# RenYurui/Global-Flow-Local-Attention

Hardware: AMD Instinct MI355X
Metric: images/sec (fwd+bwd) PoseGenerator 256x176 attn_layer=2,3 -- feature-warping hot path (higher is better)
Workload: dtype f32 (FC products: 2-term f16 splits exact to 2^-24 on f16 MFMA, f32 accumulate)

## Files before the change

### global_flow_local_attention_amd/csrc/fc_block.hip

```cpp
#include "fc_gemm.h"

namespace gfla {

static int64_t align256(int64_t v) { return (v + 255) & ~(int64_t)255; }

enum { kAmaxSrc = 0, kAmaxTgt = 1, kAmaxW = 2, kAmaxZs = 3, kAmaxZt = 4, kAmaxSlots = 8 };

enum FcConv {
  kConvDirect,
  kConvDirect16,
  kConvWino32,
  kConvWino16,
};
enum FcWgrad {
  kWgradDirect32,
  kWgradDirect16,
  kWgradWino32,
  kWgradWino16,
};
static bool fc_wgrad_wino(FcWgrad w) { return w == kWgradWino32 || w == kWgradWino16; }

struct FcPlan {
  int split;
  bool scaled;
  FcConv fwd, dgrad;
  bool pack_wf, pack_wd;
  int pack_split;
  bool pack_uf, pack_ud;
  bool dgrads_together;
  FcWgrad wgrad;
  FcWgrad wgrad_both;
  bool wgrads_together;
  bool wgrad_x32;
  bool own_scatter;
};

static FcPlan fc_plan(int64_t B, int C, int H, int W, int k, int mode) {
  (void)C;
  FcPlan P;
  P.split = fc_base_mode(mode);
  P.scaled = P.split != 0 || mode == 5;
  P.fwd = mode == 4 ? kConvWino32 : mode == 5 ? (k == 5 ? kConvDirect16 : kConvWino16) : kConvDirect;
  P.dgrad = mode == 4 ? kConvWino32 : mode == 5 ? kConvDirect16 : kConvDirect;
  P.pack_wf = P.fwd == kConvDirect || P.fwd == kConvDirect16;
  P.pack_wd = P.dgrad == kConvDirect || P.dgrad == kConvDirect16;
  P.pack_split = P.dgrad == kConvDirect16 ? 2 : P.split;
  P.pack_uf = P.fwd == kConvWino32 || P.fwd == kConvWino16;
  P.pack_ud = P.dgrad == kConvWino32;
  P.dgrads_together = fc_is_wino(mode);
  P.wgrad_x32 = mode == 1 && k == 5;
  P.wgrad = fc_is_wino(mode) || P.wgrad_x32 ? (mode == 5 && k == 5 ? kWgradWino16 : kWgradWino32)
                                            : (P.split ? kWgradDirect16 : kWgradDirect32);
  P.wgrad_both = P.wgrad_x32 ? kWgradWino16 : P.wgrad;
  P.wgrads_together = tuning(GFLA_TUNE_WINO_LAUNCH) != 2;
  const FcHalf hs = fc_half(H, W, k, true);
  P.own_scatter = tuning(GFLA_TUNE_FC_SCATTER_ATOMICS) != 1 && fc_scatter_own_rows(B, hs.Ho, hs.Wo) >= 1;
  return P;
}

struct FcLayout {
  FcPlan plan;
  FcHalf hs, ht;
  int nch_c, cpad, nt_d, KK, dw1_tiles;
  int64_t amax, xs, xt, gs, hid, wd_t, wd_s, gt, wf_t, wf_s, wu_ft, wu_fs, wu_dt, wu_ds, fwd_total;
  int64_t dzs, dzt, dw_s, dw_t, zero_bytes, zs_pk, zt_pk, dxs, dxt, b0p, dw1p, red, red_tmp, dwp, dwp2, x32, x32b, bwd_total;
};

static FcLayout fc_layout(int64_t B, int C, int H, int W, int k, int mode) {
  const bool wino = fc_is_wino(mode);
  FcLayout L;
  L.plan = fc_plan(B, C, H, W, k, mode);
  const FcPlan &P = L.plan;
  L.hs = fc_half(H, W, k, true);
  L.ht = fc_half(H, W, k, false);
  L.nch_c = (int)ceil_div(C, kFcChunk);
  L.cpad = L.nch_c * kFcChunk;
  L.nt_d = (int)ceil_div(C, kFcTN);
  L.KK = k * k;
  const int nch_h = kFcHidden / kFcChunk;
  int64_t o = 0;
  auto take = [&](int64_t bytes) {
    const int64_t at = o;
    o += align256(bytes);
    return at;
  };
  L.amax = take(kAmaxSlots * 4);
  L.xs = take(fc_packed_bytes(B, L.nch_c, L.hs.Sx, P.split));
  L.xt = take(fc_packed_bytes(B, L.nch_c, L.ht.Sx, P.split));
  L.gs = take(B * L.hs.Mg * kFcHidden * 4);
  L.hid = take(B * (int64_t)H * W * kFcHidden * 4);
// ... 279 lines not shown
static int fc_fold_both(const FcLayout &L, const unsigned char *sc, float *g_source, float *g_target, int acc_s, int64_t B, int C,
                        int H, int W, hipStream_t stream) {
  return fc_fold2(reinterpret_cast<const float *>(sc + L.dxs), g_source, L.hs, L.hs.Mdg * (int64_t)C, acc_s,
                  reinterpret_cast<const float *>(sc + L.dxt), g_target, L.ht, L.ht.Mdg * (int64_t)C, 0, B, C, H, W, stream);
}

static int fc_unpack_wgrad_both(const FcLayout &L, const unsigned char *ws, unsigned char *sc, float *g_w0, int C, int k,
                                hipStream_t stream) {
  const uint32_t *a = reinterpret_cast<const uint32_t *>(ws + L.amax);
  return fc_unpack_wgrad(reinterpret_cast<float *>(sc + L.dw_t), reinterpret_cast<float *>(sc + L.dw_s), a + kAmaxTgt, a + kAmaxSrc,
                         a + kAmaxZt, a + kAmaxZs, g_w0, C, L.cpad, k, stream);
}

static int fc_backward(void *ws_, const float *flow, const float *w1, const float *g_logits, void *scratch_,
                       float *g_source, float *g_target, float *g_flow, float *g_w0, float *g_b0, float *g_w1,
                       float *g_b1, int64_t B, int C, int H, int W, int k, float slope, int mode_, int flags,
                       hipStream_t stream) {
  if (!ws_ || !flow || !w1 || !g_logits || !scratch_) return GFLA_ERR_NULL_POINTER;
  GFLA_TRY(fc_args_ok(B, C, H, W, k, mode_));
  if (B == 0) return GFLA_OK;
  note_path(mode_ == 5 ? GFLA_PATH_FC_BWD_MODE5 : GFLA_PATH_FC_BWD_MODE0 + mode_);
  const FcLayout L = fc_layout(B, C, H, W, k, mode_);
  const FcPlan &P = L.plan;
  unsigned char *ws = static_cast<unsigned char *>(ws_), *sc = static_cast<unsigned char *>(scratch_);
  uint32_t *amax = reinterpret_cast<uint32_t *>(ws + L.amax);
  const float *hid = reinterpret_cast<const float *>(ws + L.hid);
  float *red_tmp = reinterpret_cast<float *>(sc + L.red_tmp);
  const float *gs = reinterpret_cast<const float *>(ws + L.gs);
  const bool need_s = g_source || g_w0, need_t = g_target || g_w0;
  float *dzs = need_s ? reinterpret_cast<float *>(sc + L.dzs) : nullptr;
  float *dzt = need_t ? reinterpret_cast<float *>(sc + L.dzt) : nullptr;
  float *b0p = g_b0 ? reinterpret_cast<float *>(sc + L.b0p) : nullptr;
  const int64_t tiles = ceil_div((int64_t)H * W, 64);
  const bool own = need_s && need_t && P.own_scatter;
  if (hipMemsetAsync(sc + (own ? L.dzt : 0), 0, L.zero_bytes - (own ? L.dzt : 0), stream) != hipSuccess) return GFLA_ERR_LAUNCH;
  if ((P.scaled || own) && hipMemsetAsync(amax + kAmaxZs, 0, 8, stream) != hipSuccess) return GFLA_ERR_LAUNCH;
  GFLA_TRY(fc_sample_tail_bwd(gs, flow, hid, w1, g_logits, own ? nullptr : dzs, dzt, g_flow, b0p, B, H, W, k, L.hs.Mg * kFcHidden,
                              L.hs.Wo, L.hs.Wp, L.ht.Wp, L.hs.Sz * kFcHidden, L.ht.Sz * kFcHidden, L.hs.lead, L.ht.lead, slope,
                              flags & GFLA_FC_ACCUMULATE_FLOW, stream, own ? amax + kAmaxZt : nullptr));
  if (own)
    GFLA_TRY(fc_sample_scatter_own(flow, dzt, dzs, amax + kAmaxZt, amax + kAmaxZs, B, H, W, k, L.hs.Ho, L.hs.Wo, L.hs.Wp, L.ht.Wp,
                                   L.hs.Sz * kFcHidden, L.ht.Sz * kFcHidden, L.hs.lead, L.ht.lead, L.hs.Sz, stream));
  const float *dw1p = nullptr;
  if (g_w1 || g_b1) {
    float *part = reinterpret_cast<float *>(sc + L.dw1p);
    GFLA_TRY(fc_dw1(hid, g_logits, part, B, H * W, L.KK, L.dw1_tiles, slope, stream));
    dw1p = part;
  }
  GFLA_TRY(fc_reduce_bias_w1(b0p, B * tiles, g_b0, dw1p, B * L.dw1_tiles, g_w1, g_b1, L.KK, red_tmp, stream));
  const int acc_s = (flags & GFLA_FC_ACCUMULATE_SOURCE) ? 1 : 0;
  const bool both_x = g_source && g_target;
  const bool dgrads_done = P.dgrads_together && both_x;
  if (dgrads_done) {
    if (P.dgrad == kConvDirect16 && !own)
      GFLA_TRY(fc_maxabs_multi(dzs, B * L.hs.Sz * kFcHidden, amax + kAmaxZs, dzt, B * L.ht.Sz * kFcHidden, amax + kAmaxZt, nullptr,
                               0, nullptr, stream));
    GFLA_TRY(fc_dgrad_convs(L, ws, sc, true, true, B, C, k, stream));
    GFLA_TRY(fc_fold_both(L, sc, g_source, g_target, acc_s, B, C, H, W, stream));
  }
  const bool defer = g_w0 && P.wgrad != kWgradDirect16;
  const bool wgrads_done = defer && fc_wgrad_wino(P.wgrad) && both_x && P.wgrads_together;
  const bool z_both = P.split != 0 && need_s && need_t;
  if (z_both) {
    if (!own)
      GFLA_TRY(fc_maxabs_multi(dzs, B * L.hs.Sz * kFcHidden, amax + kAmaxZs, dzt, B * L.ht.Sz * kFcHidden, amax + kAmaxZt, nullptr,
                               0, nullptr, stream));
    GFLA_TRY(fc_pack_z2(dzs, amax + kAmaxZs, sc + L.zs_pk, L.hs.Sz, dzt, amax + kAmaxZt, sc + L.zt_pk, L.ht.Sz, B, kFcHidden,
                        P.split, stream));
// ... 154 lines not shown
```

### global_flow_local_attention_amd/csrc/fc_gemm.h

```cpp
#pragma once

#include "gfla_common.h"

namespace gfla {

typedef float f32x16 __attribute__((ext_vector_type(16)));
typedef _Float16 f16x8 __attribute__((ext_vector_type(8)));
typedef short s16x4 __attribute__((ext_vector_type(4)));
typedef short s16x8 __attribute__((ext_vector_type(8)));

constexpr int kFcChunk = 16;
constexpr int kFcTN = 128;
constexpr int kFcHidden = 128;

template <int MODE>
struct Fc;
template <>
struct Fc<0> {
  static constexpr int NS = 1, ESZ = 4, REC = 64, PIECES = 4, PITCH = 80, KB = 2;
};
template <>
struct Fc<1> {
  static constexpr int NS = 1, ESZ = 2, REC = 32, PIECES = 2, PITCH = 48, KB = 1;
};
template <>
struct Fc<2> {
  static constexpr int NS = 2, ESZ = 2, REC = 32, PIECES = 2, PITCH = 48, KB = 1;
};
template <>
struct Fc<3> {
  static constexpr int NS = 3, ESZ = 2, REC = 32, PIECES = 2, PITCH = 48, KB = 1;
};

inline bool fc_is_wino(int mode) { return mode == 4 || mode == 5; }
inline int fc_base_mode(int mode) { return fc_is_wino(mode) ? 0 : mode; }
inline int fc_nsplit(int mode) { return mode == 0 ? 1 : mode; }
inline int fc_esz(int mode) { return mode == 0 ? 4 : 2; }
inline bool fc_mode_ok(int mode) { return mode >= 0 && mode <= 5; }

struct PackedDesc {
  const unsigned char *base;
  int64_t split_stride;
  int64_t batch_stride;
  int64_t chunk_stride;
  int pix_stride;
};
// ... 172 lines not shown
```

### global_flow_local_attention_amd/csrc/fc_sample.hip

```cpp
#include "fc_gemm.h"
#include "lds_plane.h"

namespace gfla {

constexpr int kSmpPix = 64;
constexpr int kSmpPitch = kFcHidden + 1;

struct Corner {
  int i00, i01, i10, i11;
  int z00, z01, z10, z11;
  float xl, xr, yt, yb;
};

template <int KS>
__device__ __forceinline__ Corner corners(float fx, float fy, int x, int y, int H, int W, int wps, int wpz = 0) {
  constexpr int LO = KS / 2, HI = KS - 1 - LO;
  const float dx = fx + (float)x, dy = fy + (float)y;
  const float fdx = floorf(dx), fdy = floorf(dy);
  Corner c;
  c.xr = dx - fdx;
  c.xl = 1.f - c.xr;
  c.yb = dy - fdy;
  c.yt = 1.f - c.yb;
  const float cx = fminf(fmaxf(fdx, -(float)(HI + 1)), (float)(W + LO));
  const float cy = fminf(fmaxf(fdy, -(float)(HI + 1)), (float)(H + LO));
  const int qx = (int)cx, qy = (int)cy;
  const int gx0 = clampi(qx, -HI, W - 1 + LO) + HI, gx1 = clampi(qx + 1, -HI, W - 1 + LO) + HI;
  const int gy0 = clampi(qy, -HI, H - 1 + LO) + HI, gy1 = clampi(qy + 1, -HI, H - 1 + LO) + HI;
  c.i00 = gy0 * wps + gx0;
  c.i01 = gy0 * wps + gx1;
  c.i10 = gy1 * wps + gx0;
  c.i11 = gy1 * wps + gx1;
  c.z00 = gy0 * wpz + gx0;
  c.z01 = gy0 * wpz + gx1;
  c.z10 = gy1 * wpz + gx0;
  c.z11 = gy1 * wpz + gx1;
  return c;
}
// ... 166 lines not shown
    tp[0] = in ? hq[j].x : 0.f, tp[1] = in ? hq[j].y : 0.f, tp[2] = in ? hq[j].z : 0.f, tp[3] = in ? hq[j].w : 0.f;
  }
#pragma unroll
  for (int j = 0; j < NW; ++j) {
    const int i = t + 256 * j;
    if (i < kFcHidden * KK) w_s[i] = wq[j];
  }
  __syncthreads();
  {
    const int p = p0 + lane;
    const bool live = p < HW;
#pragma unroll
    for (int q = 0; q < KK; ++q) gl[q] = live ? gl[q] : 0.f;
    uint32_t mx = 0;
#pragma unroll 4
    for (int o = wave; o < kFcHidden; o += 4) {
      const float pre = tile[lane * kSmpPitch + o];
      const float *w = w_s + o * KK;
      float ga = 0.f;
#pragma unroll
      for (int q = 0; q < KK; ++q) ga = fmaf(w[q], gl[q], ga);
      const float gp = pre > 0.f ? ga : ga * slope;
      tile[lane * kSmpPitch + o] = gp;
      mx = max(mx, __float_as_uint(gp) & 0x7fffffffu);
    }
    if (amax_d) {
#pragma unroll
      for (int m = 32; m >= 1; m >>= 1) mx = max(mx, (uint32_t)__shfl_xor((int)mx, m));
      if (lane == 0 && mx > __hip_atomic_load(amax_d, __ATOMIC_RELAXED, __HIP_MEMORY_SCOPE_AGENT)) atomicMax(amax_d, mx);
    }
  }
  __syncthreads();
  const float *gsb = gs + b * gs_bs;
  float *zsb = dzs ? dzs + b * zs_bs : nullptr;
  float *ztb = dzt ? dzt + b * zt_bs : nullptr;
  float s0 = 0.f, s1 = 0.f;
  int pend_t = -1, pend_b = -1;
  float pt0 = 0.f, pt1 = 0.f, pb0 = 0.f, pb1 = 0.f;
  constexpr int kWalk = kSmpPix / 4;
  const int pw0 = p0 + wave * kWalk;
  const int nwalk = max(0, min(kWalk, HW - pw0));
  float fx_l = 0.f, fy_l = 0.f;
  if ((lane & (kWalk - 1)) < nwalk) {
    fx_l = flow[(b * 2 + 0) * HW + pw0 + (lane & (kWalk - 1))];
    fy_l = flow[(b * 2 + 1) * HW + pw0 + (lane & (kWalk - 1))];
  }
  if (amax_d && __any(!(fabsf(fx_l) < INFINITY) || !(fabsf(fy_l) < INFINITY))) {
    if (lane == 0) atomicMax(amax_d, 0x7fc00000u);
  }
  Corner cn;
  float gn[8];
  auto issue = [&](int it) {
    const int p = pw0 + it;
    const int y = p / W, x = p - y * W;
    const float fx = __int_as_float(__builtin_amdgcn_readlane(__float_as_int(fx_l), it));
    const float fy = __int_as_float(__builtin_amdgcn_readlane(__float_as_int(fy_l), it));
    cn = corners<KS>(fx, fy, x, y, H, W, wps, wpz);
    if (gflow) {
      const float *g00 = gsb + (int64_t)cn.i00 * kFcHidden + lane, *g01 = gsb + (int64_t)cn.i01 * kFcHidden + lane;
      const float *g10 = gsb + (int64_t)cn.i10 * kFcHidden + lane, *g11 = gsb + (int64_t)cn.i11 * kFcHidden + lane;
      gn[0] = g00[0], gn[1] = g01[0], gn[2] = g10[0], gn[3] = g11[0];
      gn[4] = g00[64], gn[5] = g01[64], gn[6] = g10[64], gn[7] = g11[64];
    }
  };
  if (!zsb) {
    float old_x = 0.f, old_y = 0.f, res_x = 0.f, res_y = 0.f;
    if (gflow && acc_flow && lane < nwalk) {
      old_x = gflow[(b * 2 + 0) * HW + pw0 + lane];
// ... 77 lines not shown
        atomic_add(zb, pb0); atomic_add(zb + 64, pb1);
      }
      float *z00 = zsb + (int64_t)(lead_s + c.z00) * kFcHidden + lane, *z10 = zsb + (int64_t)(lead_s + c.z10) * kFcHidden + lane;
      atomic_add(z00, lt0); atomic_add(z00 + 64, lt1);
      atomic_add(z10, lb0); atomic_add(z10 + 64, lb1);
      pend_t = c.z01, pend_b = c.z11;
      pt0 = wb * d0, pt1 = wb * d1, pb0 = wd * d0, pb1 = wd * d1;
    }
    if (gflow) {
      float gx = d0 * (c.yt * (g[1] - g[0]) + c.yb * (g[3] - g[2])) + d1 * (c.yt * (g[5] - g[4]) + c.yb * (g[7] - g[6]));
      float gy = d0 * (c.xl * (g[2] - g[0]) + c.xr * (g[3] - g[1])) + d1 * (c.xl * (g[6] - g[4]) + c.xr * (g[7] - g[5]));
      gx = wave_sum_lane63(gx);
      gy = wave_sum_lane63(gy);
      if (lane == 63) {
        float *fxp = gflow + (b * 2 + 0) * HW + p, *fyp = gflow + (b * 2 + 1) * HW + p;
        *fxp = acc_flow ? *fxp + gx : gx;
        *fyp = acc_flow ? *fyp + gy : gy;
      }
    }
  }
  if (zsb && pend_t >= 0) {
    float *zt = zsb + (int64_t)(lead_s + pend_t) * kFcHidden + lane, *zb = zsb + (int64_t)(lead_s + pend_b) * kFcHidden + lane;
    atomic_add(zt, pt0); atomic_add(zt + 64, pt1);
    atomic_add(zb, pb0); atomic_add(zb + 64, pb1);
  }
  if (b0_partials) {
    bsum[wave * kFcHidden + lane] = s0;
    bsum[wave * kFcHidden + lane + 64] = s1;
    __syncthreads();
    if (t < kFcHidden)
      b0_partials[(b * gridDim.x + blockIdx.x) * kFcHidden + t] =
          (bsum[t] + bsum[kFcHidden + t]) + (bsum[2 * kFcHidden + t] + bsum[3 * kFcHidden + t]);
  }
}

static int smp_check(int64_t B, int H, int W, int k) {
  if (B < 0 || H <= 0 || W <= 0) return GFLA_ERR_BAD_SHAPE;
  if (k != 3 && k != 5) return GFLA_ERR_UNSUPPORTED;
  if (B > 65535 || (int64_t)H * W > 0x3fffffffLL) return GFLA_ERR_UNSUPPORTED;
  return GFLA_OK;
}

int fc_sample_tail_fwd(const float *gs, const float *gt, const float *flow, const float *b0, const float *w1,
                       const float *b1, float *hid, float *logits, int64_t B, int H, int W, int k, int64_t gs_bs,
                       int64_t gt_bs, int wps, int wpt, float slope, hipStream_t stream) {
  if (!gs || !gt || !flow || !w1 || !hid || !logits) return GFLA_ERR_NULL_POINTER;
  if (int rc = smp_check(B, H, W, k)) return rc;
  if (B == 0) return GFLA_OK;
  const dim3 grid((unsigned)ceil_div((int64_t)H * W, kSmpPix), (unsigned)B);
  const unsigned lds = (unsigned)((kSmpPix * kSmpPitch + kFcHidden * k * k) * sizeof(float));
  if (k == 3)
    fc_tail_fwd_kernel<3><<<grid, 256, lds, stream>>>(gs, gt, flow, b0, w1, b1, hid, logits, H, W, gs_bs, gt_bs, wps, wpt, slope);
  else
    fc_tail_fwd_kernel<5><<<grid, 256, lds, stream>>>(gs, gt, flow, b0, w1, b1, hid, logits, H, W, gs_bs, gt_bs, wps, wpt, slope);
  return launch_status();
}

int fc_sample_tail_bwd(const float *gs, const float *flow, const float *hid, const float *w1, const float *g_logits,
                       float *dzs, float *dzt, float *gflow, float *b0_partials, int64_t B, int H, int W, int k,
                       int64_t gs_bs, int wps, int wpz, int wpt, int64_t zs_bs, int64_t zt_bs, int lead_s, int lead_t,
                       float slope, int acc_flow, hipStream_t stream, uint32_t *amax_d) {
  if (!gs || !flow || !hid || !w1 || !g_logits) return GFLA_ERR_NULL_POINTER;
  if (int rc = smp_check(B, H, W, k)) return rc;
  if (B == 0) return GFLA_OK;
  const dim3 grid((unsigned)ceil_div((int64_t)H * W, kSmpPix), (unsigned)B);
  const unsigned lds = (unsigned)((kSmpPix * kSmpPitch + kFcHidden * k * k + 4 * kFcHidden) * sizeof(float));
// ... 626 lines not shown
```

### global_flow_local_attention_amd/csrc/gs_route.h

```cpp
#pragma once

#include <type_traits>

#include "agg_stream.h"
#include "be_bwd_lds.h"
#include "be_fwd_pix.h"
#include "be_fwd_wrow.h"
#include "be_tile.h"

namespace gfla {

template <int LO, int HI, typename F>
inline void k_dispatch(int k, F &&f) {
  if constexpr (LO >= HI) {
    f(std::integral_constant<int, HI>{});
  } else {
    if (k == LO) f(std::integral_constant<int, LO>{});
    else k_dispatch<LO + 1, HI>(k, f);
  }
}
#define GFLA_K_SWITCH(NAME, LO, HI, KV, ...) \
  ::gfla::k_dispatch<LO, HI>(KV, [&](auto gfla_k_) { constexpr int NAME = decltype(gfla_k_)::value; __VA_ARGS__; })
#define GFLA_WIN_SWITCH(MARGIN, ...)                                   \
  do {                                                                 \
// ... 274 lines not shown

enum class AggGaPath { kUnsupported, kStream, kLds };
struct AggGaRoute {
  AggGaPath path;
  AggStreamPlan plan;
  int G, nsuper, CS, ntiles;
  int64_t blocks, padded;
  unsigned lds_bytes;
};
inline AggGaRoute agg_ga_route(int acc_size, int64_t B, int64_t C, int64_t Hs, int64_t Ws, int64_t H, int64_t W, int k) {
  AggGaRoute r{};
  if (acc_size == 4 && agg_stream_wanted(k) && agg_stream_shape_ok(B, C, Hs, Ws, k, false) &&
      agg_stream_plan(B, C, Hs, Ws, H, W, k, r.plan))
    return r.path = AggGaPath::kStream, r;
  const int64_t ntiles = ceil_div(H * W, 512);
  int64_t G = lds_budget() / (Hs * Ws * (int64_t)acc_size);
  if (G < 1) return r;
  if (G > C) G = C;
  int64_t nsuper = 1;
  while (B * ntiles * nsuper < 4 * kNumCU && nsuper * 2 * G <= C) nsuper *= 2;
  const int64_t CS = ceil_div(C, nsuper);
  nsuper = ceil_div(C, CS);
  if (G > CS) G = CS;
  r.G = (int)G, r.nsuper = (int)nsuper, r.CS = (int)CS, r.ntiles = (int)ntiles;
  r.blocks = B * nsuper * ntiles;
  r.padded = ceil_div(r.blocks, kNumXCD) * kNumXCD;
  r.lds_bytes = (unsigned)(G * Hs * Ws * acc_size);
  if (grid_ok(r.blocks)) r.path = AggGaPath::kLds;
  return r;
}
enum class AggBwdPath { kUnsupported, kLds, kGlobal };
struct AggBwdRoute {
  AggBwdPath path;
  bool product, lds_fallback;
  PlaneGeo scatter, fallback;
  Geo global;
};
inline AggBwdRoute agg_bwd_route(int elem_size, int acc_size, bool need_src, bool need_flow, bool need_logits, bool workspace,
                                 int64_t B, int64_t C, int64_t Hs, int64_t Ws, int64_t H, int64_t W, int k) {
  AggBwdRoute r{};
  const bool half = elem_size == 2, fit = scatter_gather_planes_fit(Hs, Ws, acc_size);
  r.product = elem_size == 4 && need_src && workspace && tuning(GFLA_TUNE_AGG) != 1 &&
              (Hs * Ws * (int64_t)acc_size <= lds_budget() || (!need_flow && !need_logits));
  r.lds_fallback = r.product && fit;
  if (r.lds_fallback) r.fallback = whole_plane_bwd_route(kGoutAttn, elem_size, acc_size, true, false, B, C, Hs, Ws, H, W, k);
  if ((tuning(GFLA_TUNE_AGG) != 1 || half) && fit) {
    r.path = AggBwdPath::kLds;
    if (need_src || need_flow) {
      r.scatter = whole_plane_bwd_route(kGoutAttn, elem_size, acc_size, need_src, need_flow, B, C, Hs, Ws, H, W, k);
      if (r.scatter.G == 0) r.path = AggBwdPath::kUnsupported;
    }
  } else if (!half) {
    r.global = chunk_geometry(B, C, H * W, 32, kHalfFillWaves);
    if (grid_ok(r.global.blocks)) r.path = AggBwdPath::kGlobal;
  }
  return r;
}

}
```

### global_flow_local_attention_amd/csrc/local_attn_aggregate.hip

```cpp
#include <type_traits>

#include "gfla_common.h"
#include "gs_route.h"
#include "patch_mfma.h"
#include "rs_taps.h"

namespace gfla {

template <typename A>
__device__ __forceinline__ A exp_t(A v);
template <>
__device__ __forceinline__ float exp_t<float>(float v) { return expf(v); }
template <>
__device__ __forceinline__ double exp_t<double>(double v) { return exp(v); }

template <typename A, int K>
struct PatchTaps {
  int xL[K], xR[K], yT[K], yB[K];
  A ax[K], ay[K];
  int x0, y0;
  bool dense;

  __device__ __forceinline__ void init(A fx0, A fy0, int xf, int yf, int Hs, int Ws) {
    dense = true;
// ... 978 lines not shown
                                                   pg.lds, stream, src, flow, gout, (float *)glogits,
                                                   gflow ? attn : (const T *)nullptr, (float *)gflow, (int)C, (int)Hs, (int)Ws,
                                                   (int)H, (int)W, pg.CH, pg.CS, pg.nsuper, pg.tgroups, pg.pitch, (int)r.plan.total,
                                                   pg.tw_log2, pg.ntile)));
    }
  } else {
    GFLA_K_SWITCH(K, 1, 5, k, agg_ga_lds_kernel<T, K><<<dim3((unsigned)r.padded), dim3(512), r.lds_bytes, stream>>>(
                                  src, flow, gout, glogits, gflow ? attn : nullptr, gflow, (int)C, (int)Hs, (int)Ws, (int)H, (int)W,
                                  r.G, r.nsuper, r.CS, r.ntiles, (int)r.blocks));
  }
  int st = launch_status();
  if (st == GFLA_OK && sm && glogits) {
    const int64_t n = B * H * W;
    GFLA_K_SWITCH(K, 1, 5, k, agg_softmax_bwd_kernel<T, K><<<dim3((unsigned)ceil_div(n, kBlock)), dim3(kBlock), 0, stream>>>(
                                  attn, glogits, n, (int)(H * W)));
    st = launch_status();
  }
  return st;
}

template <typename T>
static int launch_agg_scatter(const PlaneGeo &g, const T *src, const T *flow, const T *attn, const T *gout, T *gsrc,
                              typename Num<T>::acc *gflow, int64_t B, int64_t C, int64_t Hs, int64_t Ws, int64_t H, int64_t W, int k,
                              hipStream_t stream, const unsigned *skip_stat = nullptr, unsigned skip_limit = 0) {
  int st = GFLA_OK;
  GFLA_K_SWITCH(K, 1, 5, k, st = launch_be_bwd_lds<T, K>(kGoutAttn, g, src, flow, gout, attn, gsrc, gflow, B, C, Hs, Ws, H, W, stream,
                                                         0, 0, (const T *)nullptr, skip_stat, skip_limit));
  return st;
}

template <typename T>
static int aggregate_bwd(const T *src, const T *flow, const T *attn, const T *gout, T *gsrc,
                         typename Num<T>::acc *gflow, typename Num<T>::acc *glogits, int64_t B, int64_t C, int64_t Hs, int64_t Ws, int64_t H, int64_t W,
                         int k, int sm, gfla_stream_t stream_, void *workspace = nullptr) {
  if (!src || !flow || !attn || !gout) return GFLA_ERR_NULL_POINTER;
  int st = agg_check(B, C, Hs, Ws, H, W, k);
  if (st != GFLA_OK) return st;
  if (!gsrc && !gflow && !glogits) return GFLA_OK;
  hipStream_t stream = static_cast<hipStream_t>(stream_);
  using A = typename Num<T>::acc;
  const AggBwdRoute r = agg_bwd_route((int)sizeof(T), (int)sizeof(A), gsrc != nullptr, gflow != nullptr, glogits != nullptr,
                                      workspace != nullptr, B, C, Hs, Ws, H, W, k);
  if constexpr (std::is_same<T, float>::value) {
    if (r.product) {
      if (r.lds_fallback && r.fallback.G == 0) return GFLA_ERR_UNSUPPORTED;
      const unsigned *skip_stat = nullptr;
      unsigned skip_limit = 0;
      st = agg_source_bwd_mfma(flow, attn, gout, gsrc, workspace, B, C, Hs, Ws, H, W, k, 1, r.lds_fallback ? 1 : 0, &skip_stat,
                               &skip_limit, stream);
      if (st == GFLA_OK) {
        if (r.lds_fallback && skip_limit != 0xffffffffu) {
          st = launch_agg_scatter<T>(r.fallback, src, flow, attn, gout, gsrc, (A *)nullptr, B, C, Hs, Ws, H, W, k, stream, skip_stat,
                                     skip_limit);
          if (st != GFLA_OK) return st;
        }
        if (gflow || glogits) st = launch_agg_ga<T>(src, flow, attn, gout, glogits, gflow, B, C, Hs, Ws, H, W, k, sm, stream);
        return st;
      }
      if (st != GFLA_ERR_UNSUPPORTED) return st;
    }
  }
  switch (r.path) {
    case AggBwdPath::kUnsupported: return GFLA_ERR_UNSUPPORTED;
    case AggBwdPath::kLds:
      st = GFLA_OK;
      if (gsrc || gflow) st = launch_agg_scatter<T>(r.scatter, src, flow, attn, gout, gsrc, gflow, B, C, Hs, Ws, H, W, k, stream);
      if (st == GFLA_OK && glogits)
        st = launch_agg_ga<T>(src, flow, attn, gout, glogits, (A *)nullptr, B, C, Hs, Ws, H, W, k, sm, stream);
      return st;
    case AggBwdPath::kGlobal:
      if constexpr (sizeof(T) != 2) {
        const Geo &g = r.global;
        GFLA_K_SWITCH(K, 1, 5, k, agg_bwd_kernel<T, K><<<dim3((unsigned)g.blocks), dim3(kBlock), 0, stream>>>(
                                      src, flow, attn, gout, gsrc, gflow, glogits, (int)C, (int)Hs, (int)Ws, (int)H, (int)W, sm, g.cpt,
                                      g.ncg, g.sp_blocks));
      }
      return launch_status();
  }
  return st;
}

template <typename T>
static int local_attn_source_bwd(const T *src, const T *flow, const T *gunf, const T *attn, const T *gout,
                                 T *gsrc, typename Num<T>::acc *gflow, int64_t B, int64_t C, int64_t Hs, int64_t Ws, int64_t H,
                                 int64_t W, int k, int layout, gfla_stream_t stream_) {
  using A = typename Num<T>::acc;
  if (!src || !flow || (!gunf && !(attn && gout)) || ((attn == nullptr) != (gout == nullptr))) return GFLA_ERR_NULL_POINTER;
  int st = agg_check(B, C, Hs, Ws, H, W, k);
  if (st != GFLA_OK) return st;
  if (!scatter_gather_planes_fit(Hs, Ws, sizeof(A))) return GFLA_ERR_UNSUPPORTED;
  if (!gsrc && !gflow) return GFLA_OK;
  hipStream_t stream = static_cast<hipStream_t>(stream_);
// ... 31 lines not shown
  int gfla_local_attn_aggregate_bwd_##SFX(const T *s, const T *f, const T *a, const T *go, T *gs, R *gf, R *gl,          \
                                          GFLA_SHAPE_PARAMS, int k, int sm, gfla_stream_t st) {                          \
    using E = gfla::elem_##SFX;                                                                                          \
    return gfla::aggregate_bwd<E>(gfla::as<E>(s), gfla::as<E>(f), gfla::as<E>(a), gfla::as<E>(go), gfla::as<E>(gs), gf,  \
                                  gl, GFLA_SHAPE_ARGS, k, sm, st);                                                       \
  }
#define GFLA_DEF_SOURCE_BWD(SFX, T, R)                                                                                   \
  int gfla_local_attn_source_bwd_##SFX(const T *s, const T *f, const T *gu, const T *a, const T *go, T *gs, R *gf,       \
                                       GFLA_SHAPE_PARAMS, int k, int layout, gfla_stream_t st) {                         \
    using E = gfla::elem_##SFX;                                                                                          \
    return gfla::local_attn_source_bwd<E>(gfla::as<E>(s), gfla::as<E>(f), gfla::as<E>(gu), gfla::as<E>(a),               \
                                          gfla::as<E>(go), gfla::as<E>(gs), gf, GFLA_SHAPE_ARGS, k, layout, st);         \
  }

extern "C" {
GFLA_DEF_AGGREGATE_FWD(f32, float)
GFLA_DEF_AGGREGATE_FWD(f64, double)
GFLA_DEF_AGGREGATE_FWD(bf16, uint16_t)
GFLA_DEF_AGGREGATE_FWD(f16, uint16_t)
GFLA_DEF_AGGREGATE_FWD_WS(f32, float)
GFLA_DEF_AGGREGATE_FWD_WS(bf16, uint16_t)
GFLA_DEF_AGGREGATE_FWD_WS(f16, uint16_t)
GFLA_DEF_AGGREGATE_BWD(f32, float, float)
GFLA_DEF_AGGREGATE_BWD(f64, double, double)
GFLA_DEF_SOURCE_BWD(f32, float, float)
GFLA_DEF_SOURCE_BWD(f64, double, double)
GFLA_DEF_AGGREGATE_BWD(bf16, uint16_t, float)
GFLA_DEF_AGGREGATE_BWD(f16, uint16_t, float)
GFLA_DEF_SOURCE_BWD(bf16, uint16_t, float)
GFLA_DEF_SOURCE_BWD(f16, uint16_t, float)
int gfla_local_attn_aggregate_bwd_ws_f32(const float *s, const float *f, const float *a, const float *go, float *gs,
                                         float *gf, float *gl, void *workspace, GFLA_SHAPE_PARAMS, int k, int sm,
                                         gfla_stream_t st) {
  return gfla::aggregate_bwd<float>(s, f, a, go, gs, gf, gl, GFLA_SHAPE_ARGS, k, sm, st, workspace);
}
int64_t gfla_aggregate_fwd_workspace_bytes(int64_t B, int64_t H, int64_t W, int k) {
  if (B <= 0 || H <= 0 || W <= 0 || k < 1 || k > 5) return 0;
  int64_t tiles = 0;
  for (int l = 3; l <= 5; ++l) tiles = std::max<int64_t>(tiles, gfla::ceil_div(W, 1 << l) * gfla::ceil_div(H, 64 >> l));
  return B * tiles * 64 * (int64_t)gfla::agg_record_floats(k) * 4;
}
int gfla_aggregate_fwd_geometry(int64_t B, int64_t C, int64_t Hs, int64_t Ws, int64_t H, int64_t W, int k, int64_t *out) {
  if (!out) return GFLA_ERR_NULL_POINTER;
  if (B <= 0 || C <= 0 || Hs <= 0 || Ws <= 0 || H <= 0 || W <= 0 || k < 1 || k > 5) return GFLA_ERR_BAD_SHAPE;
  if (!gfla::agg_stream_shape_ok(B, C, Hs, Ws, k, true)) return GFLA_ERR_UNSUPPORTED;
  const gfla::AggStreamGeo g = gfla::agg_stream_geometry(B, C, Hs, Ws, H, W, k);
  if (g.CH <= 0) return GFLA_ERR_UNSUPPORTED;
  const int64_t v[9] = {g.CH, g.CS, g.nsuper, g.tgroups, g.threads, g.pitch, 1 << g.tw_log2, g.ntile, g.lds};
  for (int i = 0; i < 9; ++i) out[i] = v[i];
  return GFLA_OK;
}
}
```

### global_flow_local_attention_amd/csrc/patch_mfma.hip

```cpp
#include "gfla_common.h"
#include "patch_mfma.h"
#include "rs_taps.h"

namespace gfla {

typedef float pm_f32x16 __attribute__((ext_vector_type(16)));

struct PatchEntry {
  int q;
  float v;
};

constexpr int kPmStatSlots = 32;
constexpr int kPmTile = 32;
constexpr int kPmSub = 8;
constexpr int kPmChannels = 128;
constexpr int kPmMaxNB = 6;
constexpr int kPmGPitch = 33;
constexpr int kPmEntrySlots = 40;

struct PmLayout {
  int64_t ntiles, table_bytes, rows_bytes, total;
};
static PmLayout pm_layout(int64_t B, int64_t HW, int entries) {
// ... 341 lines not shown
  while (R > 1 && R * Ws > kPmMaxNB * 32) --R;
  if (R * Ws > kPmMaxNB * 32) return PmGeo{0, 0, 0};
  return PmGeo{R, (int)ceil_div((int64_t)R * Ws, 32), (int)ceil_div(Hs, R)};
}

static bool pm_auto(bool aggregate, int64_t Ws) {
  if (tuning(GFLA_TUNE_PM) == 2) return true;
  return aggregate ? true : Ws <= 24;
}

static int64_t pm_lds_bytes(int NB, int64_t ntiles) {
  return (int64_t)(kPmTile * NB * 32 + kPmChannels * kPmGPitch) * (int64_t)sizeof(float) + ((ntiles + 7) & ~(int64_t)7) * 2;
}

static bool pm_supported(int64_t B, int64_t C, int64_t H, int64_t W, int64_t Hs, int64_t Ws) {
  if (!(B > 0 && B <= 65535 && C > 0 && Hs >= 2 && Ws >= 2 && Ws <= kPmMaxNB * 32 && Hs < 32768 && Ws < 32768 &&
        H * W <= (int64_t)kPmTile * 65535 && ceil_div(C, kPmChannels) <= 65535 && tuning(GFLA_TUNE_PM) != 1))
    return false;
  const PmGeo g = pm_geometry(B, C, (int)Hs, (int)Ws, (int)W, 0);
  return g.R > 0 && pm_lds_bytes(g.NB, ceil_div(H * W, kPmTile)) <= 64 * 1024;
}

static bool pm_g_vec(const float *G, int64_t HW) {
  return (HW & 3) == 0 && (reinterpret_cast<uintptr_t>(G) & 15) == 0;
}

template <int NB, bool VEC>
__global__ __launch_bounds__(256, NB <= 3 ? 4 : 3) void patch_scatter_mfma_kernel(
    const float *__restrict__ G, float *__restrict__ dS, const PatchEntry *__restrict__ table,
    const int2 *__restrict__ tile_rows, int C, int HW, int Hs, int Ws, int R, int ntiles, int E, int accumulate,
    const unsigned *__restrict__ stat, unsigned limit) {
  constexpr int NQ = NB * 32;
  constexpr bool kSkip = NB >= 3;
  if (pm_stat_total(stat) > limit) return;
  extern __shared__ __attribute__((aligned(16))) unsigned char gfla_smem[];
  float *wt = reinterpret_cast<float *>(gfla_smem);
  float *gt = wt + kPmTile * NQ;
  unsigned short *list = reinterpret_cast<unsigned short *>(gt + kPmChannels * kPmGPitch);
  __shared__ int s_nlist;
  __shared__ unsigned s_mask[3];
  const int t = threadIdx.x, lane = t & 63, wave = t >> 6, l31 = lane & 31, kh = lane >> 5;
  const unsigned nwg = gridDim.x * gridDim.y * gridDim.z, lin = blockIdx.x + gridDim.x * (blockIdx.y + gridDim.y * blockIdx.z);
  const unsigned xq = nwg >> 3, xr = nwg & 7u, xcd = lin & 7u;
  const unsigned id = (xcd < xr ? xcd * (xq + 1) : xr * (xq + 1) + (xcd - xr) * xq) + (lin >> 3);
  const int band = (int)(id % gridDim.x);
  const int64_t b = (id / gridDim.x) % gridDim.y;
  const int c0 = (int)(id / (gridDim.x * gridDim.y)) * kPmChannels;
  const int by0 = band * R, by1 = min(Hs, by0 + R) - 1;
  const int nq = (by1 - by0 + 1) * Ws;

  if (wave == 0) {
    const int2 *tr = tile_rows + b * ntiles;
    int n = 0;
    for (int base = 0; base < ntiles; base += 64 * kPmListBatch) {
      int2 rr[kPmListBatch];
#pragma unroll
      for (int u = 0; u < kPmListBatch; ++u) rr[u] = tr[min(base + 64 * u + lane, ntiles - 1)];
#pragma unroll
      for (int u = 0; u < kPmListBatch; ++u) {
        const int tile = base + 64 * u + lane;
        const bool f = tile < ntiles && rr[u].x <= by1 && rr[u].y >= by0;
        const unsigned long long m = __ballot(f);
        if (f) list[n + __popcll(m & ((1ull << lane) - 1ull))] = (unsigned short)tile;
        n += __popcll(m);
      }
    }
    if (lane == 0) s_nlist = n;
  }
  __syncthreads();
  const int nlist = s_nlist;

  pm_f32x16 acc[NB];
#pragma unroll
  for (int j = 0; j < NB; ++j)
#pragma unroll
    for (int r = 0; r < 16; ++r) acc[j][r] = 0.f;

  const int gc = t >> 1, gh = t & 1;
  const bool g_ok = c0 + gc < C;
  const float *g_chan = G + (b * C + min(c0 + gc, C - 1)) * (int64_t)HW;
  const int pl = t >> 3, sub = t & (kPmSub - 1);
  const PatchEntry *tab = table + (b * ntiles * kPmTile + pl) * (int64_t)E;
// ... 228 lines not shown
```

### global_flow_local_attention_amd/extractor_attn.py

```python
import torch
import torch.nn as nn
import torch.nn.functional as F
from torch.autograd import Function

from . import _lib, fc_f64, fc_mfma
from .block_extractor import BlockExtractor
from .local_attn_reshape import LocalAttnReshape

_FUSED_MAX_K = 5

VENDOR_FALLBACK = "warn"
vendor_fallback_calls = 0


class VendorFallbackError(RuntimeError):
    pass


class _SourceGradLink(object):

    def __init__(self):
        self.pending = None
        self.unfold_alive = False

# ... 270 lines not shown
        blocks = False
    else:
        u_s = self.extractor(source_c, flow_c)
        u_t = self.extractor(target_c, zero_flow)
        blocks = True
    hidden_s, hidden_t = fc_f64.Fc0F64Function.apply(conv0.weight, u_t, u_s, k, blocks)
    logits = FcTailFunction.apply(hidden_s, hidden_t, conv0.bias, conv1.weight.view(conv1.out_channels, -1), conv1.bias,
                                  _tail_slope(act), True)
    return _aggregate(source_c, flow_c, logits, last, k, link)


class FusedAttnFunction(Function):

    @staticmethod
    def forward(ctx, source, target, flow, w0, b0, w1, b1, kernel_size, slope, mode):
        k, mode = int(kernel_size), int(mode)
        fc_mfma._check(source, target, flow, w0, w1, k)
        source, target, flow = source.contiguous(), target.contiguous(), flow.contiguous()
        logits, ws, w1c = fc_mfma.forward_call(source, target, flow, w0, b0, w1, b1, k, slope, mode)
        out = torch.empty_like(source)
        attn = torch.empty_like(logits)
        _lib.aggregate_fwd(source, flow, logits, out, attn, k, True)
        ctx.save_for_backward(source, flow, attn, w1c, ws)
        ctx.dims = tuple(source.shape) + (k, float(slope), mode)
        ctx.w_shapes = (w0.shape, w1.shape, b0 is not None, b1 is not None)
        ctx.mark_non_differentiable(attn)
        return out, attn

    @staticmethod
    def backward(ctx, g_out, _g_attn):
        source, flow, attn, w1c, ws = ctx.saved_tensors
        B, C, H, W, k = ctx.dims[:5]
        need = ctx.needs_input_grad
        g_source, g_flow, g_logits = _zeros_f32(source.device, ((B, C, H, W), need[0]), ((B, 2, H, W), need[2]),
                                                (attn.shape, True))
        fc_mfma.aggregate_backward_f32(source, flow, attn, g_out.contiguous(), g_source, g_flow, g_logits, k)
        return fc_mfma.backward_call(ws, flow, w1c, g_logits, ctx.dims, ctx.w_shapes, need, flags=3, g_source=g_source,
                                     g_flow=g_flow) + (None, None, None)


def _zeros_f32(dev, *wanted_shapes):
    sizes = [(-(-int(torch.Size(shape).numel()) // 64) * 64 if wanted else 0) for shape, wanted in wanted_shapes]
    arena = torch.zeros(sum(sizes), dtype=torch.float32, device=dev)
    out, at = [], 0
    for (shape, wanted), n in zip(wanted_shapes, sizes):
        out.append(arena[at:at + torch.Size(shape).numel()].view(shape) if wanted else None)
        at += n
    return out


BF16_BACKWARD_F32_AGGREGATE = True


class FusedAttn16Function(Function):

    @staticmethod
    def forward(ctx, source, target, flow, w0, b0, w1, b1, kernel_size, slope):
        k = int(kernel_size)
        dt = source.dtype
        _lib.require_gpu(source, target, flow, w0, w1)
        B, C, H, W = source.shape
        if tuple(target.shape) != (B, C, H, W) or tuple(flow.shape) != (B, 2, H, W):
            raise ValueError("ExtractorAttn (%s): source, target and flow must share B, C and H, W" % dt)
        source, flow = source.contiguous(), flow.contiguous()
        mode = 1
        if dt == torch.float16:
            fl32 = _lib.convert_many([flow.detach()], torch.float32)[0]
            logits32, ws, w1c = fc_mfma.forward_call(source, target.detach().contiguous(), fl32, w0, b0, w1, b1, k, slope, mode)
        else:
# ... 269 lines not shown
```

### global_flow_local_attention_amd/fc_mfma.py

```python
import ctypes

import torch
from torch.autograd import Function

from . import _lib

MODES = (0, 1, 2, 3, 4, 5)
DEFAULT_MODE = 5
MODE_NAMES = {0: "f32 MFMA, direct convolution", 1: "one f16 term per operand (exact for bf16 values), f32 accumulate",
              2: "two f16 terms per operand, f32 accumulate", 3: "three f16 terms per operand, f32 accumulate",
              4: "f32 MFMA, Winograd-domain convolutions F(2x2,5x5) / F(4x4,3x3)",
              5: "two f16 terms per operand on f16 MFMA, f32 accumulate: direct kernels (k5 convolutions, data gradients) + "
                 "Winograd domain F(2x2,5x5) / F(4x4,3x3) (k3 forward, k5 weight gradient)"}


def supported(C, H, W, k, mode=DEFAULT_MODE):
    return bool(_lib.lib().gfla_fc_supported(int(C), int(H), int(W), int(k), int(mode)))


def resolve_mode(C, H, W, k, mode=None):
    mode = DEFAULT_MODE if mode is None else int(mode)
    if mode not in MODES:
        return None
    if supported(C, H, W, k, mode):
# ... 41 lines not shown
    B, C, H, W = source.shape
    w0c, w1c, b0c, b1c = _f32c(w0), _f32c(w1).reshape(k * k, 128), _f32c(b0), _f32c(b1)
    ws = torch.empty(workspace_bytes(B, C, H, W, k, mode, 0), dtype=torch.uint8, device=source.device)
    logits = torch.empty((B, k * k, H, W), dtype=torch.float32, device=source.device)
    P = _lib.ptr
    if source.dtype == torch.float16:
        assert mode == 1, "gfla_fc_forward_f16 feeds the mode-1 backward"
        _lib.call("gfla_fc_forward_f16", source, P(source), P(target), P(flow), P(w0c), P(b0c), P(w1c), P(b1c), P(ws), P(logits),
                  B, C, H, W, k, float(slope))
    else:
        _lib.call("gfla_fc_forward_f32", source, P(source), P(target), P(flow), P(w0c), P(b0c), P(w1c), P(b1c), P(ws), P(logits),
                  B, C, H, W, k, float(slope), mode)
    return logits, ws, w1c


def backward_call(ws, flow, w1c, g_logits, dims, w_shapes, need, flags=0, g_source=None, g_flow=None):
    B, C, H, W, k, slope, mode = dims
    w0_shape, w1_shape, has_b0, has_b1 = w_shapes
    dev = flow.device
    g_logits = g_logits.contiguous()

    def new(shape, wanted):
        return torch.empty(shape, dtype=torch.float32, device=dev) if wanted else None

    g = (new((B, C, H, W), need[0]) if g_source is None else g_source, new((B, C, H, W), need[1]),
         new((B, 2, H, W), need[2]) if g_flow is None else g_flow, new(w0_shape, need[3]), new((128,), need[4] and has_b0),
         new(w1_shape, need[5]), new((k * k,), need[6] and has_b1))
    scratch = torch.empty(workspace_bytes(B, C, H, W, k, mode, 1), dtype=torch.uint8, device=dev)
    _lib.call("gfla_fc_backward_f32", flow, _lib.ptr(ws), _lib.ptr(flow), _lib.ptr(w1c), _lib.ptr(g_logits),
              _lib.ptr(scratch), *[_lib.ptr(t) for t in g], B, C, H, W, k, slope, mode, flags)
    return g


def aggregate_backward_f32(source, flow, attn, g_out, g_source, g_flow, g_logits, k, apply_softmax=True):
    b, c, hs, ws = source.shape
    h, w = flow.shape[2:]
    table = _lib.scatter_workspace(source, b, h, w, (k + 1) ** 2) if g_source is not None else None
    _lib.call("gfla_local_attn_aggregate_bwd_ws_f32", source, _lib.ptr(source), _lib.ptr(flow), _lib.ptr(attn), _lib.ptr(g_out),
              _lib.ptr(g_source), _lib.ptr(g_flow), _lib.ptr(g_logits), _lib.ptr(table), b, c, hs, ws, h, w, k,
              1 if apply_softmax else 0)


class FcMfmaFunction(Function):
    @staticmethod
    def forward(ctx, source, target, flow, w0, b0, w1, b1, kernel_size, slope, mode):
        k, mode = int(kernel_size), int(mode)
        _check(source, target, flow, w0, w1, k)
        source, target, flow = source.contiguous(), target.contiguous(), flow.contiguous()
        logits, ws, w1c = forward_call(source, target, flow, w0, b0, w1, b1, k, slope, mode)
        ctx.save_for_backward(flow, w1c, ws)
        ctx.dims = tuple(source.shape) + (k, float(slope), mode)
        ctx.w_shapes = (w0.shape, w1.shape, b0 is not None, b1 is not None)
        return logits

    @staticmethod
    def backward(ctx, g_logits):
        flow, w1c, ws = ctx.saved_tensors
        return backward_call(ws, flow, w1c, g_logits, ctx.dims, ctx.w_shapes, ctx.needs_input_grad) + (None, None, None)
```

Baseline: 9812.

## Drop redundant zero-fills: overwrite source grad in aggregate bwd, zero z-pad in tail kernel

The g_source buffer is no longer zero-initialized in Python. The aggregate backward MFMA path now overwrites it instead of accumulating, and the skip path writes explicit zeros for skipped bands. The FC backward no longer memsets the whole scratch region. The sample-tail kernel writes zeros into the padding/halo cells of the dzt map it owns, and only the dzs and wgrad regions are memset when needed. The aim is to cut full-buffer memset traffic, at the cost of more complex initialization invariants that could leave stale data if any path misses a cell.

Measured after the change: 9829, median of 2. About the same (+0.2%).

```diff
diff --git a/global_flow_local_attention_amd/csrc/fc_block.hip b/global_flow_local_attention_amd/csrc/fc_block.hip
--- a/global_flow_local_attention_amd/csrc/fc_block.hip
+++ b/global_flow_local_attention_amd/csrc/fc_block.hip
@@ -56,6 +56,19 @@
   const FcHalf hs = fc_half(H, W, k, true);
   P.own_scatter = tuning(GFLA_TUNE_FC_SCATTER_ATOMICS) != 1 && fc_scatter_own_rows(B, hs.Ho, hs.Wo) >= 1;
   return P;
+}
+
+struct FcZero {
+  bool own;
+  bool dzs;
+  bool dw;
+};
+static FcZero fc_zero(const FcPlan &P, bool need_s, bool need_t) {
+  FcZero z;
+  z.own = need_s && need_t && P.own_scatter;
+  z.dzs = need_s && !z.own;
+  z.dw = P.wgrad == kWgradDirect16;
+  return z;
 }
 
 struct FcLayout {
@@ -401,8 +414,10 @@
   float *dzt = need_t ? reinterpret_cast<float *>(sc + L.dzt) : nullptr;
   float *b0p = g_b0 ? reinterpret_cast<float *>(sc + L.b0p) : nullptr;
   const int64_t tiles = ceil_div((int64_t)H * W, 64);
-  const bool own = need_s && need_t && P.own_scatter;
-  if (hipMemsetAsync(sc + (own ? L.dzt : 0), 0, L.zero_bytes - (own ? L.dzt : 0), stream) != hipSuccess) return GFLA_ERR_LAUNCH;
+  const FcZero zero = fc_zero(P, need_s, need_t);
+  const bool own = zero.own;
+  if (zero.dzs && hipMemsetAsync(sc + L.dzs, 0, L.dzt - L.dzs, stream) != hipSuccess) return GFLA_ERR_LAUNCH;
+  if (zero.dw && hipMemsetAsync(sc + L.dw_s, 0, L.zero_bytes - L.dw_s, stream) != hipSuccess) return GFLA_ERR_LAUNCH;
   if ((P.scaled || own) && hipMemsetAsync(amax + kAmaxZs, 0, 8, stream) != hipSuccess) return GFLA_ERR_LAUNCH;
   GFLA_TRY(fc_sample_tail_bwd(gs, flow, hid, w1, g_logits, own ? nullptr : dzs, dzt, g_flow, b0p, B, H, W, k, L.hs.Mg * kFcHidden,
                               L.hs.Wo, L.hs.Wp, L.ht.Wp, L.hs.Sz * kFcHidden, L.ht.Sz * kFcHidden, L.hs.lead, L.ht.lead, slope,
diff --git a/global_flow_local_attention_amd/csrc/fc_gemm.h b/global_flow_local_attention_amd/csrc/fc_gemm.h
--- a/global_flow_local_attention_amd/csrc/fc_gemm.h
+++ b/global_flow_local_attention_amd/csrc/fc_gemm.h
@@ -1,6 +1,7 @@
 #pragma once
 
 #include "gfla_common.h"
+#include "fc_tail_own.h"
 
 namespace gfla {
 
@@ -12,6 +13,7 @@
 constexpr int kFcChunk = 16;
 constexpr int kFcTN = 128;
 constexpr int kFcHidden = 128;
+static_assert(kFcZChannels == kFcHidden, "fc_tail_own.h: a pixel of the gradient map holds the hidden channels");
 
 template <int MODE>
 struct Fc;
diff --git a/global_flow_local_attention_amd/csrc/fc_sample.hip b/global_flow_local_attention_amd/csrc/fc_sample.hip
--- a/global_flow_local_attention_amd/csrc/fc_sample.hip
+++ b/global_flow_local_attention_amd/csrc/fc_sample.hip
@@ -3,7 +3,7 @@
 
 namespace gfla {
 
-constexpr int kSmpPix = 64;
+constexpr int kSmpPix = kFcTailPix;
 constexpr int kSmpPitch = kFcHidden + 1;
 
 struct Corner {
@@ -236,8 +236,7 @@
   }
   __syncthreads();
   const float *gsb = gs + b * gs_bs;
-  float *zsb = dzs ? dzs + b * zs_bs : nullptr;
-  float *ztb = dzt ? dzt + b * zt_bs : nullptr;
+  float *zsb = dzs ? dzs + b * zs_bs : nullptr, *ztb = dzt ? dzt + b * zt_bs : nullptr;
   float s0 = 0.f, s1 = 0.f;
   int pend_t = -1, pend_b = -1;
   float pt0 = 0.f, pt1 = 0.f, pb0 = 0.f, pb1 = 0.f;
@@ -381,6 +380,7 @@
       b0_partials[(b * gridDim.x + blockIdx.x) * kFcHidden + t] =
           (bsum[t] + bsum[kFcHidden + t]) + (bsum[2 * kFcHidden + t] + bsum[3 * kFcHidden + t]);
   }
+  if (ztb) fc_tail_store_zeros(ztb, (int)blockIdx.x, t, H, W, wpt, lead_t, zt_bs / kFcHidden);
 }
 
 static int smp_check(int64_t B, int H, int W, int k) {
diff --git a/global_flow_local_attention_amd/csrc/fc_tail_own.h b/global_flow_local_attention_amd/csrc/fc_tail_own.h
--- /dev/null
+++ b/global_flow_local_attention_amd/csrc/fc_tail_own.h
@@ -0,0 +1,47 @@
+#pragma once
+
+#include <stdint.h>
+
+#if defined(__HIPCC__)
+#define GFLA_HD __host__ __device__ __forceinline__
+#else
+#define GFLA_HD inline
+#endif
+
+namespace gfla {
+
+constexpr int kFcTailPix = 64;
+
+GFLA_HD int64_t fc_z_pixel(int p, int W, int wp, int lead) {
+  const int y = p / W;
+  return (int64_t)lead + (int64_t)y * wp + (p - y * W);
+}
+
+struct FcZRange {
+  int64_t lo, hi;
+};
+GFLA_HD FcZRange fc_tail_z_range(int tile, int HW, int W, int wp, int lead, int64_t Sz) {
+  const int p0 = tile * kFcTailPix, p1 = p0 + kFcTailPix;
+  return FcZRange{tile == 0 ? 0 : fc_z_pixel(p0, W, wp, lead), p1 >= HW ? Sz : fc_z_pixel(p1, W, wp, lead)};
+}
+
+GFLA_HD bool fc_z_is_data(int64_t z, int H, int W, int wp, int lead) {
+  const int64_t r = z - lead;
+  if (r < 0) return false;
+  const int64_t y = r / wp;
+  return y < H && r - y * wp < W;
+}
+
+#if defined(__HIPCC__)
+constexpr int kFcZChannels = 128;
+__device__ __forceinline__ void fc_tail_store_zeros(float *zb, int tile, int t, int H, int W, int wp, int lead, int64_t Sz) {
+  const FcZRange zr = fc_tail_z_range(tile, H * W, W, wp, lead, Sz);
+  const float4 z4 = make_float4(0.f, 0.f, 0.f, 0.f);
+  for (int64_t z = zr.lo + (t >> 5); z < zr.hi; z += 256 / 32)
+    if (!fc_z_is_data(z, H, W, wp, lead)) reinterpret_cast<float4 *>(zb + z * kFcZChannels)[t & 31] = z4;
+}
+#endif
+
+}
+
+#undef GFLA_HD
diff --git a/global_flow_local_attention_amd/csrc/gs_route.h b/global_flow_local_attention_amd/csrc/gs_route.h
--- a/global_flow_local_attention_amd/csrc/gs_route.h
+++ b/global_flow_local_attention_amd/csrc/gs_route.h
@@ -330,12 +330,13 @@
 enum class AggBwdPath { kUnsupported, kLds, kGlobal };
 struct AggBwdRoute {
   AggBwdPath path;
-  bool product, lds_fallback;
+  bool product, lds_fallback, zero_fill;
   PlaneGeo scatter, fallback;
   Geo global;
 };
 inline AggBwdRoute agg_bwd_route(int elem_size, int acc_size, bool need_src, bool need_flow, bool need_logits, bool workspace,
-                                 int64_t B, int64_t C, int64_t Hs, int64_t Ws, int64_t H, int64_t W, int k) {
+                                 int64_t B, int64_t C, int64_t Hs, int64_t Ws, int64_t H, int64_t W, int k,
+                                 bool src_uninit = false) {
   AggBwdRoute r{};
   const bool half = elem_size == 2, fit = scatter_gather_planes_fit(Hs, Ws, acc_size);
   r.product = elem_size == 4 && need_src && workspace && tuning(GFLA_TUNE_AGG) != 1 &&
@@ -352,6 +353,7 @@
     r.global = chunk_geometry(B, C, H * W, 32, kHalfFillWaves);
     if (grid_ok(r.global.blocks)) r.path = AggBwdPath::kGlobal;
   }
+  r.zero_fill = need_src && src_uninit && !r.product;
   return r;
 }
 
diff --git a/global_flow_local_attention_amd/csrc/local_attn_aggregate.hip b/global_flow_local_attention_amd/csrc/local_attn_aggregate.hip
--- a/global_flow_local_attention_amd/csrc/local_attn_aggregate.hip
+++ b/global_flow_local_attention_amd/csrc/local_attn_aggregate.hip
@@ -1034,7 +1034,7 @@
 template <typename T>
 static int aggregate_bwd(const T *src, const T *flow, const T *attn, const T *gout, T *gsrc,
                          typename Num<T>::acc *gflow, typename Num<T>::acc *glogits, int64_t B, int64_t C, int64_t Hs, int64_t Ws, int64_t H, int64_t W,
-                         int k, int sm, gfla_stream_t stream_, void *workspace = nullptr) {
+                         int k, int sm, gfla_stream_t stream_, void *workspace = nullptr, bool src_uninit = false) {
   if (!src || !flow || !attn || !gout) return GFLA_ERR_NULL_POINTER;
   int st = agg_check(B, C, Hs, Ws, H, W, k);
   if (st != GFLA_OK) return st;
@@ -1042,14 +1042,21 @@
   hipStream_t stream = static_cast<hipStream_t>(stream_);
   using A = typename Num<T>::acc;
   const AggBwdRoute r = agg_bwd_route((int)sizeof(T), (int)sizeof(A), gsrc != nullptr, gflow != nullptr, glogits != nullptr,
-                                      workspace != nullptr, B, C, Hs, Ws, H, W, k);
+                                      workspace != nullptr, B, C, Hs, Ws, H, W, k, src_uninit);
+  bool overwrite = src_uninit && gsrc != nullptr;
+  const auto zero_fill = [&]() {
+    overwrite = false;
+    return hipMemsetAsync(gsrc, 0, (size_t)(B * C * Hs * Ws) * sizeof(T), stream) == hipSuccess;
+  };
+  if (r.path == AggBwdPath::kUnsupported && !r.product) return GFLA_ERR_UNSUPPORTED;
+  if (r.zero_fill && !zero_fill()) return GFLA_ERR_LAUNCH;
   if constexpr (std::is_same<T, float>::value) {
     if (r.product) {
       if (r.lds_fallback && r.fallback.G == 0) return GFLA_ERR_UNSUPPORTED;
       const unsigned *skip_stat = nullptr;
       unsigned skip_limit = 0;
-      st = agg_source_bwd_mfma(flow, attn, gout, gsrc, workspace, B, C, Hs, Ws, H, W, k, 1, r.lds_fallback ? 1 : 0, &skip_stat,
-                               &skip_limit, stream);
+      st = agg_source_bwd_mfma(flow, attn, gout, gsrc, workspace, B, C, Hs, Ws, H, W, k, overwrite ? 0 : 1, r.lds_fallback ? 1 : 0,
+                               &skip_stat, &skip_limit, stream);
       if (st == GFLA_OK) {
         if (r.lds_fallback && skip_limit != 0xffffffffu) {
           st = launch_agg_scatter<T>(r.fallback, src, flow, attn, gout, gsrc, (A *)nullptr, B, C, Hs, Ws, H, W, k, stream, skip_stat,
@@ -1060,6 +1067,8 @@
         return st;
       }
       if (st != GFLA_ERR_UNSUPPORTED) return st;
+      if (r.path == AggBwdPath::kUnsupported) return GFLA_ERR_UNSUPPORTED;
+      if (overwrite && !zero_fill()) return GFLA_ERR_LAUNCH;
     }
   }
   switch (r.path) {
@@ -1157,7 +1166,7 @@
 int gfla_local_attn_aggregate_bwd_ws_f32(const float *s, const float *f, const float *a, const float *go, float *gs,
                                          float *gf, float *gl, void *workspace, GFLA_SHAPE_PARAMS, int k, int sm,
                                          gfla_stream_t st) {
-  return gfla::aggregate_bwd<float>(s, f, a, go, gs, gf, gl, GFLA_SHAPE_ARGS, k, sm, st, workspace);
+  return gfla::aggregate_bwd<float>(s, f, a, go, gs, gf, gl, GFLA_SHAPE_ARGS, k, sm & 1, st, workspace, (sm & 2) != 0);
 }
 int64_t gfla_aggregate_fwd_workspace_bytes(int64_t B, int64_t H, int64_t W, int k) {
   if (B <= 0 || H <= 0 || W <= 0 || k < 1 || k > 5) return 0;
diff --git a/global_flow_local_attention_amd/csrc/patch_mfma.hip b/global_flow_local_attention_amd/csrc/patch_mfma.hip
--- a/global_flow_local_attention_amd/csrc/patch_mfma.hip
+++ b/global_flow_local_attention_amd/csrc/patch_mfma.hip
@@ -397,7 +397,6 @@
     const unsigned *__restrict__ stat, unsigned limit) {
   constexpr int NQ = NB * 32;
   constexpr bool kSkip = NB >= 3;
-  if (pm_stat_total(stat) > limit) return;
   extern __shared__ __attribute__((aligned(16))) unsigned char gfla_smem[];
   float *wt = reinterpret_cast<float *>(gfla_smem);
   float *gt = wt + kPmTile * NQ;
@@ -413,6 +412,16 @@
   const int c0 = (int)(id / (gridDim.x * gridDim.y)) * kPmChannels;
   const int by0 = band * R, by1 = min(Hs, by0 + R) - 1;
   const int nq = (by1 - by0 + 1) * Ws;
+  if (pm_stat_total(stat) > limit) {
+    if (!accumulate) {
+      const int nc = min(kPmChannels, C - c0);
+      for (int i = threadIdx.x; i < nc * nq; i += 256) {
+        const int c = i / nq;
+        dS[((b * C + c0 + c) * (int64_t)Hs + by0) * Ws + (i - c * nq)] = 0.f;
+      }
+    }
+    return;
+  }
 
   if (wave == 0) {
     const int2 *tr = tile_rows + b * ntiles;
diff --git a/global_flow_local_attention_amd/extractor_attn.py b/global_flow_local_attention_amd/extractor_attn.py
--- a/global_flow_local_attention_amd/extractor_attn.py
+++ b/global_flow_local_attention_amd/extractor_attn.py
@@ -326,9 +326,10 @@
         source, flow, attn, w1c, ws = ctx.saved_tensors
         B, C, H, W, k = ctx.dims[:5]
         need = ctx.needs_input_grad
-        g_source, g_flow, g_logits = _zeros_f32(source.device, ((B, C, H, W), need[0]), ((B, 2, H, W), need[2]),
-                                                (attn.shape, True))
-        fc_mfma.aggregate_backward_f32(source, flow, attn, g_out.contiguous(), g_source, g_flow, g_logits, k)
+        g_source = torch.empty((B, C, H, W), dtype=torch.float32, device=source.device) if need[0] else None
+        g_flow, g_logits = _zeros_f32(source.device, ((B, 2, H, W), need[2]), (attn.shape, True))
+        fc_mfma.aggregate_backward_f32(source, flow, attn, g_out.contiguous(), g_source, g_flow, g_logits, k,
+                                       overwrite_source=True)
         return fc_mfma.backward_call(ws, flow, w1c, g_logits, ctx.dims, ctx.w_shapes, need, flags=3, g_source=g_source,
                                      g_flow=g_flow) + (None, None, None)
 
diff --git a/global_flow_local_attention_amd/fc_mfma.py b/global_flow_local_attention_amd/fc_mfma.py
--- a/global_flow_local_attention_amd/fc_mfma.py
+++ b/global_flow_local_attention_amd/fc_mfma.py
@@ -97,13 +97,13 @@
     return g
 
 
-def aggregate_backward_f32(source, flow, attn, g_out, g_source, g_flow, g_logits, k, apply_softmax=True):
+def aggregate_backward_f32(source, flow, attn, g_out, g_source, g_flow, g_logits, k, apply_softmax=True, overwrite_source=False):
     b, c, hs, ws = source.shape
     h, w = flow.shape[2:]
     table = _lib.scatter_workspace(source, b, h, w, (k + 1) ** 2) if g_source is not None else None
     _lib.call("gfla_local_attn_aggregate_bwd_ws_f32", source, _lib.ptr(source), _lib.ptr(flow), _lib.ptr(attn), _lib.ptr(g_out),
               _lib.ptr(g_source), _lib.ptr(g_flow), _lib.ptr(g_logits), _lib.ptr(table), b, c, hs, ws, h, w, k,
-              1 if apply_softmax else 0)
+              (1 if apply_softmax else 0) | (2 if overwrite_source else 0))
 
 
 class FcMfmaFunction(Function):
```
